# illini-robomaster/irmv_detection

Measured on AMD Instinct MI355X. Metric: end-to-end FPS (preprocess→NMS→PnP) 640×640 YOLOv8n, 1/2/4/8 MI355X, higher is better.
Workload: dtype f16

## Files before the change

irmv_detection_amd/_build.py:

```python
from __future__ import annotations

import os
import shutil
import subprocess

_HERE = os.path.dirname(os.path.abspath(__file__))
CSRC = os.path.join(_HERE, "csrc")
LIB_DIR = os.path.join(_HERE, "lib")
LIB_PATH = os.path.join(LIB_DIR, "libirmv_hip.so")
INCLUDE = os.path.join(os.path.dirname(_HERE), "include")

SOURCES = [
    ("k_pre.hip", []),
    ("k_bayer.hip", []),
    ("k_front.hip", []),
    ("k_c2f.hip", []),
    ("k_bneck.hip", []),
    ("k_kpt.hip", []),
    ("k_conv.hip", []),
    ("k_post.hip", ["-ffp-contract=off"]),
    ("k_light.hip", ["-ffp-contract=off"]),
    ("k_shuffle.hip", []),
    ("engine.cpp", ["-x", "hip"]),
]
COMMON = ["-O3", "-std=c++17", "-fPIC", "--offload-arch=gfx950", "-Wall", "-Wno-unused-function",
          "-mllvm", "-amdgpu-mfma-vgpr-form", "-I", INCLUDE]


def source_hash() -> str:
    import hashlib
    h = hashlib.sha256()
    names = sorted(set([s for s, _ in SOURCES] + ["irmv_common.hpp", "pnp_device.hpp", "numa.hpp"]))
    for n in names:
        pth = os.path.join(CSRC, n)
        if os.path.exists(pth):
            h.update(n.encode() + b"\0" + open(pth, "rb").read())
    h.update(open(os.path.join(INCLUDE, "irmv_hip.h"), "rb").read())
    h.update(" ".join(COMMON[:-2]).encode())
    for src, extra in SOURCES:
        h.update((src + " " + " ".join(extra)).encode())
    return h.hexdigest()


def hipcc() -> str:
    for cand in (shutil.which("hipcc"), "/opt/rocm/bin/hipcc"):
        if cand and os.path.exists(cand):
            return cand
    raise RuntimeError("hipcc not found: the HIP extension cannot be built")


def _stale(target: str, deps) -> bool:
# ... 49 lines not shown
```

irmv_detection_amd/csrc/engine.cpp:

```cpp
#include <hip/hip_runtime.h>

#include <algorithm>
#include <chrono>
#include <cmath>
#include <cstdio>
#include <cstring>
#include <fstream>
#include <map>
#include <mutex>
#include <set>
#include <memory>
#include <string>
#include <vector>

#include "../../include/irmv_hip.h"
#include "irmv_common.hpp"
#include "numa.hpp"

using namespace irmv;

constexpr int kLightPointsCap = 4096;

static thread_local std::string g_err;
static int fail(int code, const std::string &msg)
// ... 77 lines not shown
        const int shift = 126 - (int)(x >> 23);
        const uint32_t man = (x & 0x7fffffu) | 0x800000u;
        uint32_t h = man >> shift;
        const uint32_t rem = man & ((1u << shift) - 1u), half = 1u << (shift - 1);
        if (rem > half || (rem == half && (h & 1u))) h++;
        return (uint16_t)(sign | h);
    }
    uint32_t h = ((x >> 23) - 112u) << 10 | ((x >> 13) & 0x3ffu);
    const uint32_t rem = x & 0x1fffu;
    if (rem > 0x1000u || (rem == 0x1000u && (h & 1u))) h++;
    return (uint16_t)(sign | h);
}

struct Tensor {
    std::string name;
    void *base = nullptr;
    size_t slot_elems = 0;
    int H = 0, W = 0, C = 0;
    bool f32 = false;
    size_t esize() const { return f32 ? 4 : 2; }
    void *slot(int s) const { return static_cast<char *>(base) + (size_t)s * slot_elems * esize(); }
};

struct SegRef { int t = -1, coff = 0, C = 0, shift = 0; };

struct TuneSwitches {
    bool untuned, verbose, warn;
    bool has_s2, has_wres;
    std::string force_s2, force_wres;
    bool force_pw, force_pwn, force_cm, force_w8, force_nt8, force_pf4;
    bool no_pw, no_pwn, no_pf2, no_pf4, no_cm, no_w8, no_nt8, no_wres, no_deep;
};

enum OpKind { OP_PRE, OP_CONV0, OP_CONV, OP_POOL, OP_NMS, OP_LIGHT, OP_FRONT, OP_C2F2, OP_C2F32, OP_DW, OP_SHUF, OP_SCAN, OP_BNECK, OP_KPT3, OP_DEMOSAIC };

struct Op {
    OpKind kind;
    std::string layer;
    ConvCfg cfg{};
    ConvCfg cfg_one{};
    char kname_one[48] = {0};
    SegRef s0, s1;
    int Hin = 0, Win = 0, Hout = 0, Wout = 0, cin = 0, cout = 0, cout_pad = 0, ksteps = 0;
    int out_t = -1, out_coff = 0, res_t = -1, res_coff = 0;
    half_t *w_packed = nullptr;
    half_t *w_k16 = nullptr;
    half_t *w_lds[4] = {nullptr, nullptr, nullptr, nullptr};
    float *bias = nullptr;
    double flops = 0, bytes = 0;
    double w_bytes = 0;
    double out_bytes = 0;
    bool pair = false;
    int level = -1;
    char kname[48] = {0};
    int sub[4] = {-1, -1, -1, -1};
    int mode = 0;
    bool shortcut = false;
    int fuse_next = -1;
    bool fused_away = false;
    int group = -1;
    int bneck = -1;
    int kpt3 = -1;
    int tune_fuse[2] = {-1, -1};
};

enum StepKind { STEP_BATCH, STEP_ONE, STEP_MATERIALIZE, STEP_POST };

struct Launch {
    int op = -1, group = -1;
    bool cfg_one = false;
    bool fused = false;
    unsigned scan = 0;
    bool keys_only = false;
    bool once = false;
    std::string name, layer;
    double flops = 0, bytes = 0, launch_bytes = 0;
};

struct GraphKey {
    int first, count;
    StepKind kind;
    bool upload;
    bool operator<(const GraphKey &o) const { return std::tie(first, count, kind, upload) < std::tie(o.first, o.count, o.kind, o.upload); }
};

struct SlotGroup {
    int first = 0, count = 0;
    hipEvent_t h2d = nullptr, out = nullptr;
    hipStream_t compute = nullptr;
    bool in_flight = false;
    bool async_up = false;
};

struct irmv_engine {
    irmv_engine_cfg cfg{};
// ... 36 lines not shown
    int head_t[3] = {-1, -1, -1};
    float *head_all = nullptr;
    PnpConst *pnp_dev = nullptr;
    long long *dbg_dev = nullptr;
    std::set<std::string> lazy_tensors;
    bool fused_front = false;
    int front_tiles_x = 0, front_tiles_y = 0, front_stage_bytes = 0, front_tile_y = kFrontTileY;
    int front_v[4] = {0, 0, 0, 0};
    int front_fastx = 0, front_fx_i0 = 0, front_fx_step = 2;
    bool classical = false;
    signed char *light_labels = nullptr;
    size_t light_pool = 0;
    short *light_points = nullptr, *light_hulls = nullptr;
    float *light_boxes = nullptr;
    DevDet *light_dets_dev = nullptr, *light_dets_host = nullptr;
    float *boxes = nullptr;
    unsigned long long *keys = nullptr;
    DevDet *dets_dev = nullptr, *dets_host = nullptr, *dets_host_dev = nullptr;
    DevFrameOut *fout_dev = nullptr, *fout_host = nullptr, *fout_host_dev = nullptr;
    bool zero_copy_results = false;
    half_t *conv0_w = nullptr;
    float *conv0_b = nullptr;
    PostArgs post{};
    std::map<GraphKey, hipGraphExec_t> graphs;
    double last_detect_ms = 0;
    std::vector<uint8_t> blob;
    std::vector<LayerW> layers;
    std::vector<std::vector<uint16_t>> dequant;
    std::vector<std::vector<uint16_t>> merged_w;
    std::vector<std::vector<float>> merged_b;
    bool bneck64 = true;
    bool merge_head0 = false;
    bool kpt3 = true;
    TuneSwitches tune_sw{};

    ~irmv_engine();
};

static bool log_alloc() { static const bool on = getenv("IRMV_LOG_ALLOC") != nullptr; return on; }
static void log_range(const irmv_engine *e, const char *what, const void *p, size_t bytes)
{
    if (log_alloc()) fprintf(stderr, "[irmv alloc] engine %p %-18s [%p, %p) %zu bytes\n", (const void *)e, what, p, (const void *)((const char *)p + bytes), bytes);
}

irmv_engine::~irmv_engine()
{
    if (cfg.device >= 0) (void)hipSetDevice(cfg.device);
    if (stream) (void)hipStreamSynchronize(stream);
    for (int i = 0; i < 7; i++)
        if (extra_streams[i]) (void)hipStreamSynchronize(extra_streams[i]);
    if (h2d_stream) (void)hipStreamSynchronize(h2d_stream);
    if (dbg_dev) {
        std::vector<long long> h((size_t)cfg.num_slots * 16);
        if (hipMemcpy(h.data(), dbg_dev, h.size() * 8, hipMemcpyDeviceToHost) == hipSuccess)
            for (int s = 0; s < cfg.num_slots && s < std::max(4, atoi(getenv("IRMV_NMS_STAMPS") ? getenv("IRMV_NMS_STAMPS") : "0")); s++)
            {
                const long long *t = &h[(size_t)s * 16];
                fprintf(stderr, "[nms stamps] slot %d: keys %lld select %lld decode %lld sort %lld gather+classes %lld rows %lld walk %lld kpts %lld pnp %lld store %lld cycles; total %lld; n=%lld kept=%lld\n", s,
                        t[7] - t[0], t[8] - t[7], t[9] - t[8], t[1] - t[9], t[10] - t[1], t[2] - t[10], t[3] - t[2], t[11] - t[3], t[12] - t[11], t[4] - t[12], t[4] - t[0], t[5], t[6]);
            }
    }
    for (auto &g : graphs) (void)hipGraphExecDestroy(g.second);
    graphs.clear();
    if (log_alloc()) fprintf(stderr, "[irmv alloc] engine %p destroy: freeing %zu device ranges\n", (const void *)this, dev_allocs.size());
    for (void *p : dev_allocs) (void)hipFree(p);
    dev_allocs.clear();
// ... 339 lines not shown
    if (!e->kpt3 || e->ops.size() < 3) return IRMV_OK;
    const int i2 = (int)e->ops.size() - 1, i1 = i2 - 1, i0 = i2 - 2;
    const Op &o0 = e->ops[i0], &o1 = e->ops[i1], &o2 = e->ops[i2];
    const bool ok = o0.kind == OP_CONV && o1.kind == OP_CONV && o2.kind == OP_CONV && o1.fuse_next == i2 && o1.cfg.cin16 && o2.w_k16 &&
                    o0.cfg.ks == 3 && o0.cfg.stride == 1 && o0.cfg.act == 1 && !o0.cfg.out_f32 && !o0.cfg.cin16 && o0.cout_pad == 16 && !o0.pair && o0.res_t < 0 &&
                    o0.s1.C == 0 && o0.s0.shift == 0 && o0.w_lds[0] != nullptr && kpt3_eligible(o0.cin) && o1.s0.t == o0.out_t && o1.cin == 16 && o1.ksteps == 5 &&
                    o0.Hin == o1.Hin && o0.Win == o1.Win;
    if (!ok) return IRMV_OK;
    {
        const Tensor &xt = e->tensors[o0.s0.t];
        if ((double)e->cfg.num_slots * xt.H * xt.W * xt.C * 2.0 >= 2147483648.0) return IRMV_OK;
    }
    Op op;
    op.kind = OP_KPT3;
    op.layer = "model.22.cv4." + std::to_string(level) + " (one launch)";
    snprintf(op.kname, sizeof op.kname, "kpt3_c%d", o0.cin);
    op.sub[0] = i0; op.sub[1] = i1; op.sub[2] = i2;
    op.Hin = op.Hout = o0.Hin; op.Win = op.Wout = o0.Win;
    op.cin = o0.cin;
    op.level = level;
    op.flops = o0.flops + o1.flops + o2.flops;
    op.w_bytes = o0.w_bytes + o1.w_bytes + o2.w_bytes;
    op.out_bytes = o2.out_bytes;
    op.bytes = op.w_bytes + (o0.bytes - o0.w_bytes - o0.out_bytes) + o2.out_bytes;
    op.kpt3 = 1;
    e->lazy_tensors.insert(e->tensors[o0.out_t].name);
    e->lazy_tensors.insert(e->tensors[o1.out_t].name);
    e->ops.push_back(op);
    const int me = (int)e->ops.size() - 1;
    e->ops[i0].kpt3 = e->ops[i1].kpt3 = e->ops[i2].kpt3 = me;
    return IRMV_OK;
}

static int add_c2f(irmv_engine *e, const std::string &prefix, SegRef s0, SegRef s1, int H, int W, int c2, int n,
                   bool shortcut, int out_t)
{
    const int c = c2 / 2;
    int cat, tmp;
    TRY(new_tensor(e, prefix + ".cat", H, W, (2 + n) * c, false, &cat));
    TRY(new_tensor(e, prefix + ".tmp", H, W, c, false, &tmp));
    TRY(add_conv(e, prefix + ".cv1", s0, s1, H, W, cat, 0));
    for (int i = 0; i < n; i++) {
        const std::string m = prefix + ".m." + std::to_string(i);
        TRY(add_conv(e, m + ".cv1", SegRef{cat, (1 + i) * c, c, 0}, SegRef{}, H, W, tmp, 0));
        TRY(add_conv(e, m + ".cv2", SegRef{tmp, 0, c, 0}, SegRef{}, H, W, cat, (2 + i) * c, shortcut ? cat : -1,
                     (1 + i) * c));
    }
    TRY(add_conv(e, prefix + ".cv2", SegRef{cat, 0, (2 + n) * c, 0}, SegRef{}, H, W, out_t, 0));
    TRY(fuse_c2f32(e, prefix, n, shortcut, cat, tmp, out_t));
    if (c == 64) {
        TRY(fuse_bneck64(e, prefix, n, shortcut, cat, out_t));
        if (!e->ops.empty() && e->ops.back().kind == OP_BNECK) e->lazy_tensors.insert(e->tensors[tmp].name);
    }
    return IRMV_OK;
}

static void axis_taps(std::vector<AxisTap> &out, int dn_total, int sn, int dn, int pad, bool rotate)
{
    out.assign(dn_total, AxisTap{-1, -1, 0, 0});
    for (int d = 0; d < dn_total; d++) {
        const int r = d - pad;
        if (r < 0 || r >= dn) continue;
        const long long num = (long long)(2 * r + 1) * sn - dn, den = 2LL * dn;
        const long long fl = num >= 0 ? num / den : -((-num + den - 1) / den);
        const long long frac = num - fl * den;
        int w = (int)((frac * 2048 + dn) / den);
// ... 21 lines not shown
        }
    };
    int max_pitch = 0, max_rows = 0;
    for (int i = 0; i < *tiles_x; i++) {
        int lo, hi;
        span(tx, 4 * i * kFrontTileX - 3, 4 * kFrontTileX + 3, &lo, &hi);
        if (hi >= 0) max_pitch = std::max(max_pitch, std::min((hi + 4) & ~3, sw) - (lo & ~3));
    }
    for (int i = 0; i < *tiles_y; i++) {
        int lo, hi;
        span(ty, 4 * i * kFrontTileY - 3, 4 * kFrontTileY + 3, &lo, &hi);
        if (hi >= 0) max_rows = std::max(max_rows, hi - lo + 1);
    }
    if (max_pitch > 1023 || max_rows > 1023) return false;
    const size_t need = (size_t)max_pitch * max_rows * 4;
    *stage_bytes = std::max((int)std::min<size_t>((need + 255) & ~(size_t)255, 1u << 30), front_min_stage_bytes());
    return need <= (size_t)kFrontStageMax;
}

static int autotune_convs(irmv_engine *e);
static void finalize_head_fusion(irmv_engine *e);
static int build_head_groups(irmv_engine *e);
static void build_step_plans(irmv_engine *e);

static int build_engine(irmv_engine *e)
{
    const irmv_engine_cfg &c = e->cfg;
    const int net_w = c.net_size, net_h = c.net_height > 0 ? c.net_height : c.net_size, S = c.num_slots;
    HIP_TRY(hipSetDevice(c.device));
    HIP_TRY(hipStreamCreateWithFlags(&e->stream, hipStreamNonBlocking));
    e->num_streams = c.num_streams > 0 ? c.num_streams : (c.num_slots <= 4 ? c.num_slots : std::min(4, std::max(2, (c.num_slots + 127) / 128)));
    { const char *bn = getenv("IRMV_BNECK64"); e->bneck64 = !(bn && bn[0] == '0'); }
    { const char *kp = getenv("IRMV_KPT3"); e->kpt3 = !(kp && kp[0] == '0'); }
    if (const char *ns = getenv("IRMV_STREAMS")) e->num_streams = atoi(ns);
    e->num_streams = std::max(1, std::min({e->num_streams, 8, c.num_slots}));
    for (int i = 1; i < e->num_streams; i++) HIP_TRY(hipStreamCreateWithFlags(&e->extra_streams[i - 1], hipStreamNonBlocking));
    HIP_TRY(hipStreamCreateWithFlags(&e->h2d_stream, hipStreamNonBlocking));
    { const char *ic = getenv("IRMV_INLINE_COPIES"); e->inline_copies = ic && ic[0] == '1'; }
    { const char *gu = getenv("IRMV_GRAPH_UPLOAD"); e->graph_upload = !(gu && gu[0] == '0'); }
    e->slot_owner.assign(S, nullptr);
    e->frame_bytes = (size_t)c.src_width * c.src_height * 3;
    const bool bayer = c.src_format != IRMV_SRC_HWC8;
    e->src_bytes = bayer ? (size_t)c.src_width * c.src_height : e->frame_bytes;
    {
        const char *nv = getenv("IRMV_NUMA");
        const bool want = e->numa_node >= 0 && !(nv && nv[0] == '0');
        numa::ScopedNode scope(want ? e->numa_node : -1);
        const bool user = want && scope.policy();
        HIP_TRY(hipHostMalloc((void **)&e->src_host, e->src_bytes * S, user ? (hipHostMallocDefault | hipHostMallocNumaUser) : hipHostMallocDefault));
        log_range(e, "pinned src_host", e->src_host, e->src_bytes * S);
        memset(e->src_host, 0, e->src_bytes * S);
        if (hipHostGetDevicePointer((void **)&e->src_host_dev, e->src_host, 0) != hipSuccess) { e->src_host_dev = nullptr; (void)hipGetLastError(); }
        if (const char *uk = getenv("IRMV_UPLOAD_KERNEL")) e->upload_kernel_blocks = atoi(uk);
        e->numa_placed = user && scope.bound();
    }
    TRY(dev_alloc(e, (void **)&e->src_dev, e->frame_bytes * S));
    HIP_TRY(hipMemset(e->src_dev, 0, e->frame_bytes * S));
    TRY(dev_alloc(e, (void **)&e->rot_dev, e->frame_bytes));
    if (bayer) {
        TRY(dev_alloc(e, (void **)&e->raw_dev, e->src_bytes * S));
        HIP_TRY(hipMemset(e->raw_dev, 0, e->src_bytes * S));
        static const int ry[4] = {0, 1, 0, 1}, rx[4] = {0, 1, 1, 0};
        BayerArgs &b = e->bayer;
        b.raw_slot_bytes = e->src_bytes; b.dst_slot_bytes = e->frame_bytes;
        b.W = c.src_width; b.H = c.src_height;
        b.ry = ry[c.src_format - 1]; b.rx = rx[c.src_format - 1];
// ... 218 lines not shown
            TRY(add_conv(e, m.name, SegRef{P[i], 0, PC[i], 0}, SegRef{}, PH[i], PW[i], t_s0[i], 0));
            Op &mo = e->ops.back();
            const double real = nbr == 3 ? 144.0 : 128.0;
            mo.flops *= real / cm;
            mo.level = i;
        }
    }
    for (int b = 0; b < nbr; b++)
        for (int i = 0; i < 3; i++) {
            const std::string pre = std::string("model.22.") + br[b] + "." + std::to_string(i);
            const std::string tn = std::string("22.") + br[b] + "." + std::to_string(i);
            int t1 = -1, t2;
            TRY(new_tensor(e, tn + ".1", PH[i], PW[i], mid[b], false, &t2));
            if (e->merge_head0) {
                TRY(add_conv(e, pre + ".1", SegRef{t_s0[i], coff0[b], mid[b], 0}, SegRef{}, PH[i], PW[i], t2, 0));
            } else {
                TRY(new_tensor(e, tn + ".0", PH[i], PW[i], mid[b], false, &t1));
                TRY(add_conv(e, pre + ".0", SegRef{P[i], 0, PC[i], 0}, SegRef{}, PH[i], PW[i], t1, 0));
                TRY(add_conv(e, pre + ".1", SegRef{t1, 0, mid[b], 0}, SegRef{}, PH[i], PW[i], t2, 0));
            }
            TRY(add_conv(e, pre + ".2", SegRef{t2, 0, mid[b], 0}, SegRef{}, PH[i], PW[i], e->head_t[i], off[b]));
            for (size_t k = e->ops.size() - (e->merge_head0 ? 2 : 3); k < e->ops.size(); k++) e->ops[k].level = i;
            {
                const int i1 = (int)e->ops.size() - 2, i2 = i1 + 1;
                const Op &o1 = e->ops[i1], &o2 = e->ops[i2];
                const char *fh = getenv("IRMV_FUSED_HEAD");
                if (!(fh && fh[0] == '0') && o1.cout == 64 && o1.cin % 32 == 0 && o1.pair && o1.res_t < 0 && o1.cfg.stride == 1 &&
                    o2.cin == 64 && o2.ksteps == 2 && o2.cfg.ks == 1 && o2.cfg.out_f32 && o2.cfg.act == 0 && (o2.cout_pad == 16 || o2.cout_pad == 64))
                    e->ops[i1].fuse_next = i2;
                if (!(fh && fh[0] == '0') && o1.cfg.cin16 && o1.cout_pad == 16 && !o1.pair && o1.res_t < 0 && o1.cfg.stride == 1 && o1.cfg.act == 1 && o2.w_k16)
                    e->ops[i1].fuse_next = i2;
            }
            if (b == 2 && !e->merge_head0) TRY(fuse_kpt3(e, i));
        }

    TRY(dev_alloc(e, (void **)&e->boxes, (size_t)S * e->A * 16));
    TRY(dev_alloc(e, (void **)&e->keys, (size_t)S * e->A * e->nc * 8));
    { const char *sp = getenv("IRMV_SPLIT_SCAN"); e->split_scan = !(sp && sp[0] == '0'); }
    if (e->split_scan) {
        TRY(dev_alloc(e, (void **)&e->cand_counts, (size_t)S * sizeof(int)));
        HIP_TRY(hipMemset(e->cand_counts, 0, (size_t)S * sizeof(int)));
    }
    TRY(dev_alloc(e, (void **)&e->dets_dev, (size_t)S * c.max_det * sizeof(DevDet)));
    TRY(dev_alloc(e, (void **)&e->fout_dev, (size_t)S * sizeof(DevFrameOut)));
    HIP_TRY(hipMemset(e->dets_dev, 0, (size_t)S * c.max_det * sizeof(DevDet)));
    HIP_TRY(hipMemset(e->fout_dev, 0, (size_t)S * sizeof(DevFrameOut)));
    HIP_TRY(hipHostMalloc((void **)&e->dets_host, (size_t)S * c.max_det * sizeof(DevDet), hipHostMallocMapped | hipHostMallocCoherent));
    HIP_TRY(hipHostMalloc((void **)&e->fout_host, (size_t)S * sizeof(DevFrameOut), hipHostMallocMapped | hipHostMallocCoherent));
    HIP_TRY(hipHostGetDevicePointer((void **)&e->dets_host_dev, e->dets_host, 0));
    HIP_TRY(hipHostGetDevicePointer((void **)&e->fout_host_dev, e->fout_host, 0));
    log_range(e, "pinned dets_host", e->dets_host, (size_t)S * c.max_det * sizeof(DevDet));
    log_range(e, "pinned fout_host", e->fout_host, (size_t)S * sizeof(DevFrameOut));
    memset(e->dets_host, 0, (size_t)S * c.max_det * sizeof(DevDet));
    memset(e->fout_host, 0, (size_t)S * sizeof(DevFrameOut));
    if (e->split_scan) {
        Op op; op.kind = OP_SCAN; op.layer = "scan_decode"; snprintf(op.kname, sizeof op.kname, "scan_decode");
        op.bytes = (double)e->A * 64.0; e->ops.push_back(op);
    }
    { Op op; op.kind = OP_NMS; op.layer = "decode_nms_kpt_pnp"; snprintf(op.kname, sizeof op.kname, "nms_pnp");
      op.bytes = (double)e->A * 64.0; e->ops.push_back(op); }
    if (c.point_source == IRMV_POINTS_KEYPOINT_HEAD && e->nk < 8) return fail(IRMV_ERR_MODEL, "point_source = keypoint head, but the model has none");
    e->classical = c.point_source == IRMV_POINTS_CLASSICAL || (c.point_source == IRMV_POINTS_AUTO && e->nk < 8);
    { const char *z = getenv("IRMV_ZERO_COPY_RESULTS"); e->zero_copy_results = !e->classical && !(z && z[0] == '0'); }
    if (e->classical) {
        Op op; op.kind = OP_LIGHT; op.layer = "extract_armors"; snprintf(op.kname, sizeof op.kname, "light_extract");
        e->ops.push_back(op);
// ... 199 lines not shown
    }
    if (cfg->net_size < 64 || cfg->net_size % 32 != 0 || cfg->net_size > 2048) return fail(IRMV_ERR_ARG, "net_size must be a multiple of 32 in [64, 2048]");
    if (cfg->net_height != 0 && (cfg->net_height < 64 || cfg->net_height % 32 != 0 || cfg->net_height > 2048))
        return fail(IRMV_ERR_ARG, "net_height must be 0 (square) or a multiple of 32 in [64, 2048]");
    if (cfg->src_width < 2 || cfg->src_height < 2 || cfg->src_width > 4096) return fail(IRMV_ERR_ARG, "src size out of range (width <= 4096)");
    if (cfg->num_slots < 1 || cfg->num_slots > 256) return fail(IRMV_ERR_ARG, "num_slots must be 1..256");
    if (cfg->max_det < 1 || cfg->max_det > IRMV_MAX_DET_CAP) return fail(IRMV_ERR_ARG, "max_det must be 1..256");
    if (cfg->pre_nms_cap < 1 || cfg->pre_nms_cap > IRMV_CAND_CAP) return fail(IRMV_ERR_ARG, "pre_nms_cap must be 1..8192");
    if (!(cfg->score_thr > 0.f && cfg->score_thr < 1.f)) return fail(IRMV_ERR_ARG, "score_thr must be in (0, 1)");
    if (cfg->armor_size != IRMV_ARMOR_SMALL && cfg->armor_size != IRMV_ARMOR_LARGE) return fail(IRMV_ERR_ARG, "bad armor_size");
    if (cfg->point_source < 0 || cfg->point_source > 2) return fail(IRMV_ERR_ARG, "bad point_source");
    int ndev = 0;
    HIP_TRY(hipGetDeviceCount(&ndev));
    if (cfg->device < 0 || cfg->device >= ndev) return fail(IRMV_ERR_HIP, "no such HIP device");
    std::unique_ptr<irmv_engine> e(new irmv_engine);
    e->cfg = *cfg;
    if (e->cfg.net_height == 0) e->cfg.net_height = e->cfg.net_size;
    {
        int cus = 0;
        if (hipDeviceGetAttribute(&cus, hipDeviceAttributeMultiprocessorCount, cfg->device) == hipSuccess && cus > 0) e->num_cus = cus;
        int node = -1;
        if (hipDeviceGetAttribute(&node, hipDeviceAttributeHostNumaId, cfg->device) == hipSuccess) e->numa_node = node;
        else (void)hipGetLastError();
    }
    int rc = load_blob(e.get());
    e->cfg.weights_path = nullptr;
    e->cfg.weights_blob = nullptr;
    if (rc) return rc;
    rc = build_engine(e.get());
    if (rc) return rc;
    rc = autotune_convs(e.get());
    if (rc) return rc;
    finalize_head_fusion(e.get());
    rc = build_head_groups(e.get());
    if (rc) return rc;
    build_step_plans(e.get());
    rc = choose_sync_launch(e.get());
    if (rc) return rc;
    *out = e.release();
    return IRMV_OK;
}

extern "C" int irmv_engine_sync_launch(const irmv_engine *e) { return e ? e->sync_launch : 0; }

extern "C" void irmv_engine_destroy(irmv_engine *e) { delete e; }
extern "C" int irmv_engine_num_slots(const irmv_engine *e) { return e ? e->cfg.num_slots : 0; }
extern "C" int irmv_engine_max_det(const irmv_engine *e) { return e ? e->cfg.max_det : 0; }
extern "C" int irmv_engine_num_streams(const irmv_engine *e) { return e ? e->num_streams : 0; }
extern "C" int irmv_engine_num_anchors(const irmv_engine *e) { return e ? e->A : 0; }
extern "C" int irmv_engine_net_dims(const irmv_engine *e, int *width, int *height)
{
    if (!e || !width || !height) return fail(IRMV_ERR_ARG, "engine/width/height is null");
    *width = e->cfg.net_size; *height = e->cfg.net_height;
    return IRMV_OK;
}
extern "C" int irmv_engine_numa_node(const irmv_engine *e) { return e ? e->numa_node : -1; }
extern "C" int irmv_engine_numa_placed(const irmv_engine *e) { return e && e->numa_placed ? 1 : 0; }

extern "C" int irmv_numa_device_node(int device, int *node)
{
    if (!node) return fail(IRMV_ERR_ARG, "node is null");
    int v = -1;
    if (hipDeviceGetAttribute(&v, hipDeviceAttributeHostNumaId, device) != hipSuccess) {
        (void)hipGetLastError();
        v = -1;
    }
// ... 376 lines not shown
        g1.push_back(find_op("model.22.s0." + si));
        const int c2 = find_op("model.22.cv2." + si + ".1"), c3 = find_op("model.22.cv3." + si + ".1");
        g2.push_back(c2); g2.push_back(c3);
        g2_fused = g2_fused && c2 >= 0 && c3 >= 0 && e->ops[c2].fuse_next >= 0 && e->ops[c3].fuse_next >= 0;
        if (kpt) { g3.push_back(find_op("model.22.cv4." + si + ".1")); g4.push_back(find_op("model.22.cv4." + si + ".2")); }
    }
    try_group(g1, 0, {1, 2}, "head_s0");
    if (g2_fused) try_group(g2, 0, {4}, "head_s1+1x1");
    if (kpt) {
        const size_t before = e->head_groups.size();
        try_group(g3, 1, {1}, "head_kpt1");
        bool k16 = false;
        for (int i : g4) k16 = k16 || i < 0 || e->ops[i].w_k16 != nullptr;
        if (e->head_groups.size() > before && !k16) try_group(g4, 1, {1}, "head_kpt2");
    }
    HIP_TRY(hipStreamSynchronize(e->stream));
    return IRMV_OK;
}

static void build_step_plans(irmv_engine *e)
{
    for (int k = STEP_BATCH; k <= STEP_POST; k++) {
        const bool one = k == STEP_ONE, mat = k == STEP_MATERIALIZE, post = k == STEP_POST, step = !mat && !post;
        auto emits = [&](const Op &op) { return step && e->emit_scan && is_cls_final_carrier(op); };
        for (int i = 0; i < (int)e->ops.size(); i++) {
            const Op &op = e->ops[i];
            if (post && op.kind != OP_NMS && op.kind != OP_LIGHT && op.kind != OP_SCAN) continue;
            if (op.kind == OP_SCAN && e->emit_scan && !post) continue;
            const bool grouped = one && op.kind == OP_CONV && op.group >= 0;
            if (grouped && e->head_groups[op.group].members[0] != i) continue;
            const bool bneck = one && e->bneck64;
            if (op.kind == OP_BNECK ? !bneck : (op.bneck >= 0 && bneck)) continue;
            if (op.kind == OP_KPT3 ? !step : (op.kpt3 >= 0 && step)) continue;
            if (mat ? !(op.fused_away || op.fuse_next >= 0 || ((op.bneck >= 0 || op.kpt3 >= 0) && op.kind == OP_CONV)) : op.fused_away) continue;
            Launch l; l.op = i;
            l.once = op.kind == OP_LIGHT || (e->split_scan && (op.kind == OP_SCAN || op.kind == OP_NMS));
            l.keys_only = op.kind == OP_NMS && ((e->emit_scan && !post) || (post && e->post_keys_only));
            l.layer = op.layer;
            if (grouped) {
                const irmv_engine::HeadGroup &g = e->head_groups[op.group];
                l.group = op.group;
                l.name = g.name;
                l.layer += " ... (" + std::to_string(g.members.size()) + " convs)";
                for (size_t m = 0; m < g.members.size(); m++) {
                    const Op &mo = e->ops[g.members[m]];
                    if (emits(mo)) l.scan |= 1u << m;
                    l.flops += mo.flops + (mo.fuse_next >= 0 ? e->ops[mo.fuse_next].flops : 0.0);
                    l.bytes += mo.bytes;
                }
            } else {
                l.cfg_one = op.kind == OP_CONV && (one || mat) && stream_share(e, e->cfg.num_slots) > 1;
                l.fused = !mat && op.fuse_next >= 0;
                l.scan = emits(op) ? 1u : 0u;
                l.name = l.cfg_one ? op.kname_one : op.kname;
                const Op *nx = l.fused ? &e->ops[op.fuse_next] : nullptr;
                l.flops = op.flops + (nx ? nx->flops : 0.0);
                l.launch_bytes = op.w_bytes + (nx ? nx->w_bytes : 0.0);
                l.bytes = op.bytes + (nx ? nx->out_bytes - op.out_bytes + nx->w_bytes : 0.0) - l.launch_bytes;
            }
            e->plans[k].push_back(l);
        }
    }
}

struct EvRec { hipEvent_t a = nullptr, b = nullptr; };
constexpr int kProfileRepeat = 4;

static void fill_conv_args(const irmv_engine *e, const Op &op, int first, int count, ConvArgs &a, bool fused)
{
    a = ConvArgs{};
    auto seg = [&](const SegRef &s) {
        ConvSeg cs{nullptr, 0, 0, 0};
        if (s.t < 0 || s.C == 0) return cs;
        const Tensor &t = e->tensors[s.t];
        cs.p = static_cast<const half_t *>(t.slot(first)) + s.coff;
        cs.ld = t.C;
        cs.C = s.C;
        cs.shift = s.shift;
        return cs;
    };
    a.s0 = seg(op.s0);
    a.s1 = seg(op.s1);
    a.Hin = op.Hin; a.Win = op.Win; a.Hout = op.Hout; a.Wout = op.Wout;
    a.M = count * op.Hout * op.Wout;
    a.Cin = op.cin;
    a.w = op.w_packed;
// ... 158 lines not shown
        case OP_BNECK: {
            const Op &m1 = e->ops[op.sub[0]], &m2 = e->ops[op.sub[1]];
            const Tensor &ct = e->tensors[op.res_t];
            BneckArgs a{};
            a.yin = static_cast<const half_t *>(ct.slot(first)) + m1.s0.coff; a.yin_ld = ct.C;
            a.ynext = static_cast<half_t *>(ct.slot(first)) + m2.out_coff; a.ynext_ld = ct.C;
            a.cat = static_cast<const half_t *>(ct.slot(first)); a.cat_ld = ct.C;
            a.H = op.Hin; a.W = op.Win;
            a.tiles_x = (op.Win + kBneckTile - 1) / kBneckTile; a.tiles_y = (op.Hin + kBneckTile - 1) / kBneckTile;
            a.w_m1 = m1.w_lds[0]; a.b_m1 = m1.bias; a.w_m2 = m2.w_lds[0]; a.b_m2 = m2.bias;
            int ks2 = 6;
            if (op.sub[2] >= 0) {
                const Op &c2 = e->ops[op.sub[2]];
                const Tensor &ot = e->tensors[c2.out_t];
                a.out = static_cast<half_t *>(ot.slot(first)) + c2.out_coff; a.out_ld = ot.C;
                a.w_cv2 = c2.w_packed; a.b_cv2 = c2.bias;
                ks2 = c2.ksteps;
            }
            if (!launch_bneck64(op.mode, ks2, op.shortcut, a, count, s)) return fail(IRMV_ERR_ARG, "no fused bottleneck kernel for " + op.layer);
            break;
        }
        case OP_KPT3: {
            const Op &o0 = e->ops[op.sub[0]], &o1 = e->ops[op.sub[1]], &o2 = e->ops[op.sub[2]];
            const Tensor &xt = e->tensors[o0.s0.t], &ht = e->tensors[o2.out_t];
            Kpt3Args a{};
            a.x = static_cast<const half_t *>(xt.slot(first)) + o0.s0.coff; a.x_ld = xt.C;
            a.H = op.Hin; a.W = op.Win;
            a.tiles_x = (op.Win + kKpt3Tile - 1) / kKpt3Tile; a.tiles_y = (op.Hin + kKpt3Tile - 1) / kKpt3Tile;
            a.w1 = o0.w_lds[0]; a.b1 = o0.bias;
            a.w2 = o1.w_packed; a.b2 = o1.bias;
            a.w3 = o2.w_k16; a.b3 = o2.bias;
            a.out = static_cast<float *>(ht.slot(first)) + o2.out_coff; a.out_ld = ht.C;
            if (!launch_kpt3(a, op.cin, count, s)) return fail(IRMV_ERR_ARG, "no fused keypoint-branch kernel for " + op.layer);
            break;
        }
        case OP_DW: {
            DwArgs a;
            const Tensor &xt = e->tensors[op.s0.t], &ot = e->tensors[op.out_t];
            a.x = static_cast<const half_t *>(xt.slot(first)) + op.s0.coff; a.x_ld = xt.C;
            a.y = static_cast<half_t *>(ot.slot(first)) + op.out_coff; a.y_ld = ot.C;
            a.w = op.w_packed; a.b = op.bias;
            a.Hin = op.Hin; a.Win = op.Win; a.Hout = op.Hout; a.Wout = op.Wout; a.C = op.cout; a.stride = op.cfg.stride;
            launch_dwconv3x3(a, count, s);
            break;
        }
        case OP_SHUF: {
            ShufArgs a;
            const Tensor &at = e->tensors[op.s0.t], &bt = e->tensors[op.s1.t], &ot = e->tensors[op.out_t];
            a.a = static_cast<const half_t *>(at.slot(first)) + op.s0.coff; a.a_ld = at.C;
            a.b = static_cast<const half_t *>(bt.slot(first)) + op.s1.coff; a.b_ld = bt.C;
            a.out = static_cast<half_t *>(ot.slot(first)); a.out_ld = ot.C;
            a.bc = op.s0.C;
            a.pixels = (size_t)count * op.Hin * op.Win;
            launch_shuffle_cat(a, s);
            break;
        }
        case OP_CONV0: {
            Conv0Args a;
            a.x = static_cast<const half_t *>(e->tensors[op.s0.t].slot(first));
            a.y = static_cast<half_t *>(e->tensors[op.out_t].slot(first));
            a.w = e->conv0_w; a.b = e->conv0_b; a.net_w = net_w; a.net_h = net_h; a.batch = count;
            launch_conv0(a, s);
            break;
        }
        case OP_CONV: {
            const unsigned scan = rep == n - 1 ? l.scan : 0u;
// ... 708 lines not shown
```

irmv_detection_amd/csrc/irmv_common.hpp:

```cpp
#pragma once

#include <hip/hip_runtime.h>

#include <cstdint>
#include <cstdlib>

namespace irmv {

typedef _Float16 half_t;
typedef _Float16 half8 __attribute__((ext_vector_type(8)));
typedef _Float16 half4 __attribute__((ext_vector_type(4)));
typedef float f32x4 __attribute__((ext_vector_type(4)));

constexpr float kActScale = 1.44269504088896341f;
constexpr float kActUnscale = 0.693147180559945309f;
typedef unsigned int u32x4_t __attribute__((ext_vector_type(4)));
__device__ __forceinline__ float silu_rcp(float y) { return __builtin_amdgcn_rcpf(1.0f + __builtin_amdgcn_exp2f(-y)); }
__device__ __forceinline__ unsigned int silu_pack2(float y0, float y1)
{
    const float r0 = silu_rcp(y0), r1 = silu_rcp(y1);
    unsigned int o;
    asm("v_fma_mixlo_f16 %0, %1, %2, 0" : "=v"(o) : "v"(y0), "v"(r0));
    asm("v_fma_mixhi_f16 %0, %1, %2, 0" : "+v"(o) : "v"(y1), "v"(r1));
    return o;
// ... 165 lines not shown
    const half_t *yin;
    int yin_ld;
    half_t *ynext;
    int ynext_ld;
    const half_t *cat;
    int cat_ld;
    half_t *out;
    int out_ld;
    int H, W, tiles_x, tiles_y;
    const half_t *w_m1, *w_m2;
    const float *b_m1, *b_m2;
    const half_t *w_cv2;
    const float *b_cv2;
};
size_t bneck64_lds_bytes(int mode, int ks2);
bool launch_bneck64(int mode, int ks2, bool shortcut, const BneckArgs &a, int batch, hipStream_t s);

constexpr int kKpt3Tile = 10;
struct Kpt3Args {
    const half_t *x;
    int x_ld;
    int H, W, tiles_x, tiles_y;
    const half_t *w1;
    const float *b1;
    const half_t *w2;
    const float *b2;
    const half_t *w3;
    const float *b3;
    float *out;
    int out_ld;
};
bool kpt3_eligible(int cin);
bool launch_kpt3(const Kpt3Args &a, int cin, int batch, hipStream_t s);

struct ConvArgs {
    ConvSeg s0, s1;
    int Hin, Win;
    int Hout, Wout;
    int M;
    int Cin;
    const half_t *w;
    const float *bias;
    void *out;
    int out_ld;
    const half_t *res;
    int res_ld;
    int cout_pad;
    int ksteps;
    int pair;
    const half_t *w2;
    const float *bias2;
    float *out2;
    int out2_ld, n2;
    unsigned long long *scan_keys;
    int *scan_counts;
    float scan_thr;
    int scan_nc, scan_abase, scan_key_cap;
};

constexpr int kMultiMax = 6;
struct LdsMember {
    ConvArgs a;
    const half_t *wl;
    int tiles_x, tiles_y, twc_log2, patch_bytes, batch, tile2d;
    int gx, gy;
};
// ... 110 lines not shown
```

Measured before the change: 60090.

## Fuse level-0 Detect box and class branches into one three-conv kernel

Adds a fused kernel that runs both Detect head branches (cv2 and cv3) at level 0 in one launch. Each workgroup loads a 20x20 halo tile, does two 3x3 64-channel convs in LDS and then the 1x1 output conv with score scanning, all in a single pass. The intermediate activations are marked lazy, so they are not written to and re-read from global memory. In exchange the kernel uses a large LDS footprint with one workgroup per CU, recomputes the halo, and is active by default only for the batched step and non-forced tune settings.

Measured after the change: 59120, median of 2. 1.6% lower.

```diff
diff --git a/irmv_detection_amd/_build.py b/irmv_detection_amd/_build.py
--- a/irmv_detection_amd/_build.py
+++ b/irmv_detection_amd/_build.py
@@ -17,6 +17,7 @@
     ("k_c2f.hip", []),
     ("k_bneck.hip", []),
     ("k_kpt.hip", []),
+    ("k_head2.hip", []),
     ("k_conv.hip", []),
     ("k_post.hip", ["-ffp-contract=off"]),
     ("k_light.hip", ["-ffp-contract=off"]),
diff --git a/irmv_detection_amd/csrc/engine.cpp b/irmv_detection_amd/csrc/engine.cpp
--- a/irmv_detection_amd/csrc/engine.cpp
+++ b/irmv_detection_amd/csrc/engine.cpp
@@ -133,7 +133,7 @@
     bool no_pw, no_pwn, no_pf2, no_pf4, no_cm, no_w8, no_nt8, no_wres, no_deep;
 };
 
-enum OpKind { OP_PRE, OP_CONV0, OP_CONV, OP_POOL, OP_NMS, OP_LIGHT, OP_FRONT, OP_C2F2, OP_C2F32, OP_DW, OP_SHUF, OP_SCAN, OP_BNECK, OP_KPT3, OP_DEMOSAIC };
+enum OpKind { OP_PRE, OP_CONV0, OP_CONV, OP_POOL, OP_NMS, OP_LIGHT, OP_FRONT, OP_C2F2, OP_C2F32, OP_DW, OP_SHUF, OP_SCAN, OP_BNECK, OP_KPT3, OP_DEMOSAIC, OP_HEAD2 };
 
 struct Op {
     OpKind kind;
@@ -162,6 +162,7 @@
     int group = -1;
     int bneck = -1;
     int kpt3 = -1;
+    int head2 = -1;
     int tune_fuse[2] = {-1, -1};
 };
 
@@ -264,6 +265,7 @@
     bool bneck64 = true;
     bool merge_head0 = false;
     bool kpt3 = true;
+    bool head2 = true;
     TuneSwitches tune_sw{};
 
     ~irmv_engine();
@@ -669,6 +671,73 @@
     return IRMV_OK;
 }
 
+static int find_conv(const irmv_engine *e, const std::string &layer)
+{
+    for (size_t i = 0; i < e->ops.size(); i++)
+        if (e->ops[i].kind == OP_CONV && e->ops[i].layer == layer) return (int)i;
+    return -1;
+}
+
+static int add_head2(irmv_engine *e, int level)
+{
+    if (!e->head2) return IRMV_OK;
+    const std::string si = std::to_string(level);
+    int idx[2][3];
+    for (int b = 0; b < 2; b++)
+        for (int k = 0; k < 3; k++)
+            if ((idx[b][k] = find_conv(e, std::string(b ? "model.22.cv3." : "model.22.cv2.") + si + "." + std::to_string(k))) < 0) return IRMV_OK;
+    const Op &x0 = e->ops[idx[0][0]];
+    for (int b = 0; b < 2; b++) {
+        const Op &o0 = e->ops[idx[b][0]], &o1 = e->ops[idx[b][1]], &o2 = e->ops[idx[b][2]];
+        auto conv64 = [&](const Op &o) {
+            return o.cfg.ks == 3 && o.cfg.stride == 1 && o.cfg.act == 1 && !o.cfg.out_f32 && o.cin == 64 && o.cout == 64 && o.cout_pad == 64 && o.pair &&
+                   o.res_t < 0 && o.s1.C == 0 && o.s0.shift == 0 && o.w_lds[2] != nullptr && o.Hin == o.Hout && o.Win == o.Wout && o.Hin == x0.Hin && o.Win == x0.Win;
+        };
+        const bool ok = conv64(o0) && conv64(o1) && o0.s0.t == x0.s0.t && o0.s0.coff == x0.s0.coff && o1.s0.t == o0.out_t && o1.s0.coff == 0 &&
+                        o1.fuse_next == idx[b][2] && o2.cout_pad == (b ? 16 : 64);
+        if (!ok) return IRMV_OK;
+    }
+    {
+        const Tensor &xt = e->tensors[x0.s0.t];
+        if ((double)e->cfg.num_slots * xt.H * xt.W * xt.C * 2.0 >= 2147483648.0) return IRMV_OK;
+    }
+    Op op;
+    op.kind = OP_HEAD2;
+    op.layer = "model.22.cv2." + si + "+cv3." + si;
+    snprintf(op.kname, sizeof op.kname, "head2_c64");
+    op.sub[0] = idx[0][0]; op.sub[1] = idx[0][1]; op.sub[2] = idx[1][0]; op.sub[3] = idx[1][1];
+    op.Hin = op.Hout = x0.Hin; op.Win = op.Wout = x0.Win;
+    op.cin = x0.cin;
+    op.level = level;
+    for (int b = 0; b < 2; b++)
+        for (int k = 0; k < 3; k++) {
+            const Op &o = e->ops[idx[b][k]];
+            op.flops += o.flops;
+            op.w_bytes += o.w_bytes;
+        }
+    op.out_bytes = e->ops[idx[0][2]].out_bytes + e->ops[idx[1][2]].out_bytes;
+    op.bytes = op.w_bytes + (x0.bytes - x0.w_bytes - x0.out_bytes) + op.out_bytes;
+    op.head2 = 0;
+    e->ops.push_back(op);
+    return IRMV_OK;
+}
+
+static void finalize_head2(irmv_engine *e)
+{
+    const TuneSwitches &t = e->tune_sw;
+    const bool forced = t.has_s2 || t.has_wres || t.force_pw || t.force_pwn || t.force_cm || t.force_w8 || t.force_nt8 || t.force_pf4;
+    for (int i = 0; i < (int)e->ops.size(); i++) {
+        Op &op = e->ops[i];
+        if (op.kind != OP_HEAD2) continue;
+        const int f2 = e->ops[op.sub[1]].fuse_next, f3 = e->ops[op.sub[3]].fuse_next;
+        op.head2 = !forced && f2 >= 0 && f3 >= 0 && e->ops[f2].cout_pad == 64 && e->ops[f3].cout_pad == 16 ? 1 : 0;
+        if (!op.head2) continue;
+        for (int k = 0; k < 4; k++) e->ops[op.sub[k]].head2 = i;
+        e->lazy_tensors.insert(e->tensors[e->ops[op.sub[0]].out_t].name);
+        e->lazy_tensors.insert(e->tensors[e->ops[op.sub[2]].out_t].name);
+    }
+}
+
 static int add_c2f(irmv_engine *e, const std::string &prefix, SegRef s0, SegRef s1, int H, int W, int c2, int n,
                    bool shortcut, int out_t)
 {
@@ -756,6 +825,7 @@
     e->num_streams = c.num_streams > 0 ? c.num_streams : (c.num_slots <= 4 ? c.num_slots : std::min(4, std::max(2, (c.num_slots + 127) / 128)));
     { const char *bn = getenv("IRMV_BNECK64"); e->bneck64 = !(bn && bn[0] == '0'); }
     { const char *kp = getenv("IRMV_KPT3"); e->kpt3 = !(kp && kp[0] == '0'); }
+    { const char *h2 = getenv("IRMV_HEAD2"); e->head2 = !(h2 && h2[0] == '0'); }
     if (const char *ns = getenv("IRMV_STREAMS")) e->num_streams = atoi(ns);
     e->num_streams = std::max(1, std::min({e->num_streams, 8, c.num_slots}));
     for (int i = 1; i < e->num_streams; i++) HIP_TRY(hipStreamCreateWithFlags(&e->extra_streams[i - 1], hipStreamNonBlocking));
@@ -1040,6 +1110,7 @@
                     e->ops[i1].fuse_next = i2;
             }
             if (b == 2 && !e->merge_head0) TRY(fuse_kpt3(e, i));
+            if (b == 1 && i == 0 && !e->merge_head0) TRY(add_head2(e, i));
         }
 
     TRY(dev_alloc(e, (void **)&e->boxes, (size_t)S * e->A * 16));
@@ -1305,6 +1376,7 @@
     rc = autotune_convs(e.get());
     if (rc) return rc;
     finalize_head_fusion(e.get());
+    finalize_head2(e.get());
     rc = build_head_groups(e.get());
     if (rc) return rc;
     build_step_plans(e.get());
@@ -1747,7 +1819,8 @@
             const bool bneck = one && e->bneck64;
             if (op.kind == OP_BNECK ? !bneck : (op.bneck >= 0 && bneck)) continue;
             if (op.kind == OP_KPT3 ? !step : (op.kpt3 >= 0 && step)) continue;
-            if (mat ? !(op.fused_away || op.fuse_next >= 0 || ((op.bneck >= 0 || op.kpt3 >= 0) && op.kind == OP_CONV)) : op.fused_away) continue;
+            if (op.kind == OP_HEAD2 ? !(k == STEP_BATCH && op.head2 == 1) : (op.head2 >= 0 && k == STEP_BATCH)) continue;
+            if (mat ? !(op.fused_away || op.fuse_next >= 0 || ((op.bneck >= 0 || op.kpt3 >= 0 || op.head2 >= 0) && op.kind == OP_CONV)) : op.fused_away) continue;
             Launch l; l.op = i;
             l.once = op.kind == OP_LIGHT || (e->split_scan && (op.kind == OP_SCAN || op.kind == OP_NMS));
             l.keys_only = op.kind == OP_NMS && ((e->emit_scan && !post) || (post && e->post_keys_only));
@@ -1766,7 +1839,7 @@
             } else {
                 l.cfg_one = op.kind == OP_CONV && (one || mat) && stream_share(e, e->cfg.num_slots) > 1;
                 l.fused = !mat && op.fuse_next >= 0;
-                l.scan = emits(op) ? 1u : 0u;
+                l.scan = emits(op) || (op.kind == OP_HEAD2 && step && e->emit_scan) ? 1u : 0u;
                 l.name = l.cfg_one ? op.kname_one : op.kname;
                 const Op *nx = l.fused ? &e->ops[op.fuse_next] : nullptr;
                 l.flops = op.flops + (nx ? nx->flops : 0.0);
@@ -1991,6 +2064,28 @@
             a.w3 = o2.w_k16; a.b3 = o2.bias;
             a.out = static_cast<float *>(ht.slot(first)) + o2.out_coff; a.out_ld = ht.C;
             if (!launch_kpt3(a, op.cin, count, s)) return fail(IRMV_ERR_ARG, "no fused keypoint-branch kernel for " + op.layer);
+            break;
+        }
+        case OP_HEAD2: {
+            const Op &x0 = e->ops[op.sub[0]];
+            const Tensor &xt = e->tensors[x0.s0.t];
+            Head2Args a{};
+            a.x = static_cast<const half_t *>(xt.slot(first)) + x0.s0.coff; a.x_ld = xt.C;
+            a.H = op.Hin; a.W = op.Win;
+            a.tiles_x = (op.Win + kHead2Tile - 1) / kHead2Tile; a.tiles_y = (op.Hin + kHead2Tile - 1) / kHead2Tile;
+            const unsigned scan = rep == n - 1 ? l.scan : 0u;
+            for (int b = 0; b < 2; b++) {
+                const Op &o0 = e->ops[op.sub[2 * b]], &o1 = e->ops[op.sub[2 * b + 1]];
+                ConvArgs ca;
+                fill_conv_args(e, o1, first, count, ca, true);
+                if (b == 1 && scan) scan_args_for(e, o1, pa, ca);
+                Head2Branch &h = a.br[b];
+                h.w1 = o0.w_lds[2]; h.b1 = o0.bias; h.w2 = o1.w_lds[2]; h.b2 = o1.bias;
+                h.w3 = ca.w2; h.b3 = ca.bias2; h.out = ca.out2; h.out_ld = ca.out2_ld;
+                h.scan_keys = ca.scan_keys; h.scan_counts = ca.scan_counts; h.scan_thr = ca.scan_thr;
+                h.scan_nc = ca.scan_nc; h.scan_abase = ca.scan_abase; h.scan_key_cap = ca.scan_key_cap;
+            }
+            if (!launch_head2(a, count, e->num_cus, s)) return fail(IRMV_ERR_ARG, "no fused Detect-branch kernel for " + op.layer);
             break;
         }
         case OP_DW: {
diff --git a/irmv_detection_amd/csrc/irmv_common.hpp b/irmv_detection_amd/csrc/irmv_common.hpp
--- a/irmv_detection_amd/csrc/irmv_common.hpp
+++ b/irmv_detection_amd/csrc/irmv_common.hpp
@@ -221,6 +221,27 @@
 };
 bool kpt3_eligible(int cin);
 bool launch_kpt3(const Kpt3Args &a, int cin, int batch, hipStream_t s);
+
+constexpr int kHead2Tile = 16;
+struct Head2Branch {
+    const half_t *w1, *w2;
+    const float *b1, *b2;
+    const half_t *w3;
+    const float *b3;
+    float *out;
+    int out_ld;
+    unsigned long long *scan_keys;
+    int *scan_counts;
+    float scan_thr;
+    int scan_nc, scan_abase, scan_key_cap;
+};
+struct Head2Args {
+    const half_t *x;
+    int x_ld;
+    int H, W, tiles_x, tiles_y;
+    Head2Branch br[2];
+};
+bool launch_head2(const Head2Args &a, int batch, int num_cus, hipStream_t s);
 
 struct ConvArgs {
     ConvSeg s0, s1;
diff --git a/irmv_detection_amd/csrc/k_head2.hip b/irmv_detection_amd/csrc/k_head2.hip
--- /dev/null
+++ b/irmv_detection_amd/csrc/k_head2.hip
@@ -0,0 +1,259 @@
+#include <mutex>
+
+#include "irmv_common.hpp"
+
+namespace irmv {
+
+namespace {
+constexpr int HT = kHead2Tile;
+constexpr int R1 = HT + 2, R1N = R1 * R1;
+constexpr int R0 = HT + 4, R0N = R0 * R0;
+constexpr int PS = 96;
+constexpr int P0 = R0N * PS;
+constexpr int P1 = R1N * PS;
+constexpr int NTH = 512;
+constexpr int NJ1 = 6;
+constexpr int NJ2 = 2;
+constexpr int NPC = (R0N * 8 + NTH - 1) / NTH;
+constexpr int RING = 4;
+constexpr int W2N = 18 * 4 * 64;
+constexpr size_t kLdsW2 = (size_t)2 * P0;
+constexpr size_t kLdsW3 = kLdsW2 + (size_t)W2N * 16;
+constexpr size_t kLdsB3 = kLdsW3 + (size_t)8 * 64 * 16;
+constexpr size_t kLds = kLdsB3 + 64 * 4;
+static_assert(P1 <= P0, "the stage-1 plane fits where the input region was");
+static_assert(kLds <= 160 * 1024, "one workgroup per CU");
+static_assert(R1N <= 21 * 16 && R1N > 20 * 16 && 4 * NJ1 >= 21, "stage 1 is 21 pixel tiles");
+static_assert(HT == 8 * NJ2, "stage 2: eight waves, two output rows each");
+static_assert(W2N % NTH == 0, "stage-2 weights: whole pieces per thread");
+typedef unsigned int u32x4 __attribute__((ext_vector_type(4)));
+}
+
+template <int N3>
+__device__ __forceinline__ void head2_body(const Head2Args &a, const Head2Branch &b, int batch, int ipw, int tile, int grp)
+{
+    extern __shared__ __attribute__((aligned(16))) uint8_t smem[];
+    uint8_t *s_x = smem;
+    half8 *s_w2 = reinterpret_cast<half8 *>(smem + kLdsW2);
+    half8 *s_w3 = reinterpret_cast<half8 *>(smem + kLdsW3);
+    float *s_b3 = reinterpret_cast<float *>(smem + kLdsB3);
+    const int tid = threadIdx.x, lane = tid & 63;
+    const int wave = __builtin_amdgcn_readfirstlane(tid >> 6);
+    const int g = lane >> 4, r = lane & 15;
+    const int img0 = grp * ipw, nimg = min(ipw, batch - img0);
+    const int tyi = tile / a.tiles_x, txi = tile - tyi * a.tiles_x;
+    const int oy0 = tyi * HT, ox0 = txi * HT;
+    const int H = a.H, W = a.W;
+
+    int src[NPC];
+    static_assert(NTH % 8 == 0, "a thread's pieces share their eighth: piece i lands at dst0 + i * (NTH / 8) pixels");
+    const int dst0 = ((tid & 7) >> 2) * P0 + (tid >> 3) * PS + (tid & 3) * 16;
+    const bool last_piece = tid + (NPC - 1) * NTH < R0N * 8;
+#pragma unroll
+    for (int i = 0; i < NPC; i++) {
+        const int e = tid + i * NTH, px = e >> 3, q = e & 7;
+        const int ly = px / R0, lx = px - ly * R0;
+        const int gy = oy0 - 2 + ly, gx = ox0 - 2 + lx;
+        const bool in = e < R0N * 8 && (unsigned)gy < (unsigned)H && (unsigned)gx < (unsigned)W;
+        src[i] = in ? (((img0 * H + gy) * W + gx) * a.x_ld + q * 8) * 2 : 0x7fffffff;
+    }
+    const int img_stride = H * W * a.x_ld * 2;
+    const auto rs_x = __builtin_amdgcn_make_buffer_rsrc(const_cast<half_t *>(a.x), 0, batch * img_stride, 0x00020000);
+    const auto rs_w = __builtin_amdgcn_make_buffer_rsrc(const_cast<half_t *>(b.w1), 0, 18 * 4 * 1024, 0x00020000);
+    u32x4 v[NPC];
+    auto issue_x = [&](int im) {
+        const int off = __builtin_amdgcn_readfirstlane(im * img_stride);
+#pragma unroll
+        for (int i = 0; i < NPC; i++) v[i] = __builtin_bit_cast(u32x4, __builtin_amdgcn_raw_buffer_load_b128(rs_x, src[i], off, 0));
+    };
+    auto write_x = [&]() {
+#pragma unroll
+        for (int i = 0; i < NPC; i++)
+            if (i + 1 < NPC || last_piece) *reinterpret_cast<u32x4 *>(s_x + dst0 + i * (NTH / 8) * PS) = v[i];
+    };
+
+    const int q1 = wave >> 1, u1 = wave & 1;
+    int p1[NJ1], b1off[NJ1];
+#pragma unroll
+    for (int j = 0; j < NJ1; j++) {
+        const int p = (q1 + 4 * j) * 16 + r;
+        p1[j] = p < R1N ? p : -1;
+        const int pc = p < R1N ? p : 0, py = pc / R1, px = pc - py * R1;
+        b1off[j] = (py * R0 + px) * PS + g * 16;
+    }
+    auto load_a1 = [&](int k, int n) { return __builtin_bit_cast(half8, __builtin_amdgcn_raw_buffer_load_b128(rs_w, lane * 16, (k * 4 + 2 * u1 + n) * 1024, 0)); };
+
+    issue_x(0);
+    __builtin_amdgcn_sched_barrier(0);
+    half8 A1[RING][2];
+#pragma unroll
+    for (int k = 0; k < RING; k++) { A1[k][0] = load_a1(k, 0); A1[k][1] = load_a1(k, 1); }
+    {
+        constexpr int WPT = W2N / NTH;
+        half8 t[WPT];
+        const half8 *w2p = reinterpret_cast<const half8 *>(b.w2);
+#pragma unroll
+        for (int i = 0; i < WPT; i++) t[i] = w2p[tid + i * NTH];
+        const half8 t3 = reinterpret_cast<const half8 *>(b.w3)[tid < N3 * 128 ? tid : 0];
+        const float tb = b.b3[tid < N3 * 16 ? tid : 0];
+#pragma unroll
+        for (int i = 0; i < WPT; i++) s_w2[tid + i * NTH] = t[i];
+        if (tid < N3 * 128) s_w3[tid] = t3;
+        if (tid < N3 * 16) s_b3[tid] = tb;
+    }
+    __builtin_amdgcn_sched_barrier(0);
+
+    int b2off[NJ2];
+#pragma unroll
+    for (int j = 0; j < NJ2; j++) b2off[j] = ((wave + 8 * j) * R1 + r) * PS + g * 16;
+
+    for (int im = 0; im < nimg; im++) {
+        write_x();
+        __syncthreads();
+
+        f32x4 acc1[NJ1][2];
+#pragma unroll
+        for (int n = 0; n < 2; n++) {
+            const f32x4 b0 = *reinterpret_cast<const f32x4 *>(b.b1 + u1 * 32 + g * 8 + n * 4);
+#pragma unroll
+            for (int j = 0; j < NJ1; j++) acc1[j][n] = b0;
+        }
+        half8 B1[NJ1];
+#pragma unroll
+        for (int k = 0; k < 18; k++) {
+            const int c = k / 9, tap = k - c * 9, kh = tap / 3, kw = tap - kh * 3;
+            const int off = c * P0 + (kh * R0 + kw) * PS;
+#pragma unroll
+            for (int j = 0; j < NJ1; j++) B1[j] = *reinterpret_cast<const half8 *>(s_x + b1off[j] + off);
+#pragma unroll
+            for (int j = 0; j < NJ1; j++)
+#pragma unroll
+                for (int n = 0; n < 2; n++) acc1[j][n] = __builtin_amdgcn_mfma_f32_16x16x32_f16(A1[k % RING][n], B1[j], acc1[j][n], 0, 0, 0);
+            __builtin_amdgcn_sched_barrier(0);
+            if (k + RING < 18) {
+                A1[k % RING][0] = load_a1(k + RING, 0);
+                A1[k % RING][1] = load_a1(k + RING, 1);
+            }
+            __builtin_amdgcn_sched_barrier(0);
+        }
+        __syncthreads();
+#pragma unroll
+        for (int j = 0; j < NJ1; j++) {
+            if (p1[j] >= 0) {
+                const int py = p1[j] / R1, px = p1[j] - py * R1;
+                const int gy = oy0 - 1 + py, gx = ox0 - 1 + px;
+                half8 o = (half8){0, 0, 0, 0, 0, 0, 0, 0};
+                if ((unsigned)gy < (unsigned)H && (unsigned)gx < (unsigned)W)
+                    o = silu_pack8(acc1[j][0][0], acc1[j][0][1], acc1[j][0][2], acc1[j][0][3], acc1[j][1][0], acc1[j][1][1], acc1[j][1][2], acc1[j][1][3]);
+                *reinterpret_cast<half8 *>(s_x + u1 * P1 + p1[j] * PS + g * 16) = o;
+            }
+        }
+        __syncthreads();
+        issue_x(im + 1 < nimg ? im + 1 : im);
+
+        f32x4 acc2[NJ2][4];
+#pragma unroll
+        for (int nt = 0; nt < 4; nt++) {
+            const f32x4 b0 = *reinterpret_cast<const f32x4 *>(b.b2 + (nt >> 1) * 32 + g * 8 + (nt & 1) * 4);
+#pragma unroll
+            for (int j = 0; j < NJ2; j++) acc2[j][nt] = b0;
+        }
+#pragma unroll
+        for (int k = 0; k < 18; k++) {
+            const int c = k / 9, tap = k - c * 9, kh = tap / 3, kw = tap - kh * 3;
+            const half8 *s_wc = s_w2 + (c * 9 + tap) * 256 + lane;
+            const int off = c * P1 + (kh * R1 + kw) * PS;
+            half8 A2[4], B2[NJ2];
+#pragma unroll
+            for (int nt = 0; nt < 4; nt++) A2[nt] = s_wc[nt * 64];
+#pragma unroll
+            for (int j = 0; j < NJ2; j++) B2[j] = *reinterpret_cast<const half8 *>(s_x + b2off[j] + off);
+#pragma unroll
+            for (int j = 0; j < NJ2; j++)
+#pragma unroll
+                for (int nt = 0; nt < 4; nt++) acc2[j][nt] = __builtin_amdgcn_mfma_f32_16x16x32_f16(A2[nt], B2[j], acc2[j][nt], 0, 0, 0);
+        }
+        __builtin_amdgcn_sched_barrier(0);
+#pragma unroll
+        for (int k = 0; k < RING; k++) { A1[k][0] = load_a1(k, 0); A1[k][1] = load_a1(k, 1); }
+        __builtin_amdgcn_sched_barrier(0);
+
+        const int im_abs = img0 + im;
+#pragma unroll
+        for (int j = 0; j < NJ2; j++) {
+            const int gy = oy0 + wave + 8 * j, gx = ox0 + r;
+            const bool valid = gy < H && gx < W;
+            const int mloc = gy * W + gx;
+            half8 ov0 = silu_pack8(acc2[j][0][0], acc2[j][0][1], acc2[j][0][2], acc2[j][0][3], acc2[j][1][0], acc2[j][1][1], acc2[j][1][2], acc2[j][1][3]);
+            half8 ov1 = silu_pack8(acc2[j][2][0], acc2[j][2][1], acc2[j][2][2], acc2[j][2][3], acc2[j][3][0], acc2[j][3][1], acc2[j][3][2], acc2[j][3][3]);
+            mfma_operand_fence(ov0, ov1);
+#pragma unroll
+            for (int t2 = 0; t2 < N3; t2++) {
+                f32x4 c2 = (f32x4){0.f, 0.f, 0.f, 0.f};
+                c2 = __builtin_amdgcn_mfma_f32_16x16x32_f16(s_w3[(t2 * 2 + 0) * 64 + lane], ov0, c2, 0, 0, 0);
+                c2 = __builtin_amdgcn_mfma_f32_16x16x32_f16(s_w3[(t2 * 2 + 1) * 64 + lane], ov1, c2, 0, 0, 0);
+                const int co = t2 * 16 + g * 4;
+                const f32x4 bb = *reinterpret_cast<const f32x4 *>(s_b3 + co);
+                const f32x4 v2 = (f32x4){c2[0] * kActUnscale + bb[0], c2[1] * kActUnscale + bb[1], c2[2] * kActUnscale + bb[2], c2[3] * kActUnscale + bb[3]};
+                if (valid) *reinterpret_cast<f32x4 *>(b.out + ((size_t)im_abs * H * W + mloc) * b.out_ld + co) = v2;
+                if (b.scan_keys) {
+                    bool hit = false;
+#pragma unroll
+                    for (int i = 0; i < 4; i++) hit = hit || (valid && co + i < b.scan_nc && v2[i] > b.scan_thr);
+                    if (hit) {
+                        const int an = b.scan_abase + mloc;
+#pragma unroll
+                        for (int i = 0; i < 4; i++) {
+                            if (co + i < b.scan_nc && v2[i] > b.scan_thr) {
+                                const int idx = atomicAdd(&b.scan_counts[im_abs], 1);
+                                const unsigned int uu = __float_as_uint(v2[i]);
+                                const unsigned int ord = (uu & 0x80000000u) ? ~uu : (uu | 0x80000000u);
+                                if (idx >= 0 && idx < b.scan_key_cap)
+                                    b.scan_keys[(size_t)im_abs * b.scan_key_cap + idx] =
+                                        ((unsigned long long)ord << 32) | (unsigned long long)(0xffffffffu - (unsigned int)(an * b.scan_nc + co + i));
+                            }
+                        }
+                    }
+                }
+            }
+        }
+        __syncthreads();
+    }
+}
+
+__global__ __launch_bounds__(NTH) __attribute__((amdgpu_waves_per_eu(2))) void head2_kernel(Head2Args a, int batch, int ipw, int xcd)
+{
+    const int id = blockIdx.x, x = id & 7, j = id >> 3, br = j & 1, id2 = (j >> 1) * 8 + x;
+    const int tiles = a.tiles_x * a.tiles_y, groups = (batch + ipw - 1) / ipw;
+    if (id2 >= tiles * groups) return;
+    int tile, grp;
+    tile_image(id2, tiles, groups, xcd, tile, grp);
+    if (br == 0) head2_body<4>(a, a.br[0], batch, ipw, tile, grp);
+    else head2_body<1>(a, a.br[1], batch, ipw, tile, grp);
+}
+
+static std::mutex g_head2_attr_mu;
+
+bool launch_head2(const Head2Args &a, int batch, int num_cus, hipStream_t s)
+{
+    const int tiles = a.tiles_x * a.tiles_y;
+    if (tiles <= 0 || batch <= 0 || a.H > a.tiles_y * HT || a.W > a.tiles_x * HT) return false;
+    int ipw = 1;
+    while (ipw < batch && 2LL * tiles * ((batch + ipw - 1) / ipw) > num_cus) ipw++;
+    const int groups = (batch + ipw - 1) / ipw;
+    const int ids = (tiles * groups + 7) / 8 * 8;
+    {
+        static unsigned long long attr_done = 0;
+        int dev = 0;
+        (void)hipGetDevice(&dev);
+        std::lock_guard<std::mutex> lk(g_head2_attr_mu);
+        if (!(attr_done & (1ull << (dev & 63)))) {
+            if (hipFuncSetAttribute(reinterpret_cast<const void *>(head2_kernel), hipFuncAttributeMaxDynamicSharedMemorySize, (int)kLds) != hipSuccess) return false;
+            attr_done |= 1ull << (dev & 63);
+        }
+    }
+    hipLaunchKernelGGL(head2_kernel, dim3(2 * ids), dim3(NTH), kLds, s, a, batch, ipw, xcd_image_order());
+    return true;
+}
+
+}
```
